# yangbang18/CARE

Measured on AMD Instinct MI355X. Metric: captions/sec (greedy), higher is better.
Workload: dtype bf16; 1 GPU; MSRVTT Transformer/base task=Base feats=ViT modality=ami greedy (BASELINE.json configs[1]): [B,28,128]+[B,28,2048]+[B,28,512] fp32 feats, d=512, V=10547, 29 decoder steps; config_name=msrvtt_base_ami, global_batch=32768, lanes=1, parallelism=batch-sharded dp1 (no data-path collective; all-gather of results), hip_graph=True, absorbed_cross_attention=True, lean_encode=True

## Files before the change

### care_amd/_lib.py

```python
import ctypes
import os
from ctypes import c_char_p, c_float, c_int, c_int64, c_uint64, c_void_p

import torch

CARE_F32, CARE_BF16 = 0, 1
ACT_NONE, ACT_RELU, ACT_GELU = 0, 1, 2
ACT_CODES = {"linear": ACT_NONE, "relu": ACT_RELU, "gelu": ACT_GELU}
ABI_VERSION = 24

_ERRORS = {-1: "CARE_EINVAL (null pointer / bad size)", -2: "CARE_EALIGN (alignment)",
           -3: "CARE_ESHAPE (unsupported shape)", -4: "CARE_EDTYPE (unknown dtype/activation)"}

LIB_PATH = os.environ.get("CARE_HIP_LIB") or os.path.join(os.path.dirname(os.path.abspath(__file__)), "libcare_hip.so")
VARIANT_H16 = {"": "bf16", "f16": "fp16"}

_P, _I, _L, _F, _U = c_void_p, c_int, c_int64, c_float, c_uint64
SIGNATURES = {
    "care_gemm": [_P, _L, _P, _I, _P, _P, _L, _I, _P, _L, _I, _I, _I, _I, _I, _I, _P],
    "care_split3_weight": [_P, _P, _I, _I, _P],
    "care_gemm_split3": [_P, _L, _P, _P, _P, _L, _I, _I, _I, _P],
    "care_gemm_argmax": [_P, _L, _P, _I, _P, _P, _P, _I, _I, _I, _P],
    "care_gemm_bf16": [_P, _L, _I, _P, _P, _P, _L, _I, _P, _L, _I, _I, _I, _I, _I, _I, _P],
    "care_gemm_argmax_bf16": [_P, _L, _I, _P, _P, _P, _P, _P, _P, _I, _I, _I, _P],
    "care_gemm_tile": [_P, _L, _P, _P, _P, _L, _I, _P, _L, _I, _I, _I, _I, _I, _I, _P],
    "care_split2_act": [_P, _L, _P, _I, _I, _P],
    "care_gemm_tile_split3": [_P, _P, _P, _P, _L, _I, _P, _L, _I, _I, _I, _I, _I, _I, _P],
    "care_gemm_tile_split3_argmax": [_P, _P, _P, _P, _P, _I, _I, _I, _P],
    "care_absmax": [_P, _L, _I, _I, _P, _P],
    "care_split_pieces": [_P, _L, _I, _I, _I, _I, _I, _P, _I, _P, _P],
    "care_gemm_tile_split3_scaled": [_P, _P, _P, _P, _L, _I, _I, _I, _P, _P, _I, _P],
    "care_gemm_tile_batched": [_P, _L, _L, _P, _L, _L, _P, _I, _P, _L, _L, _I, _I, _I, _I, _I, _P],
    "care_gemm_tile_argmax": [_P, _L, _P, _P, _P, _P, _P, _P, _I, _I, _I, _P],
    "care_score_partials": [_P, _P, _P, _P, _I, _P, _P, _I, _P],
    "care_label_logits": [_P, _L, _P, _P, _P, _I, _I, _I, _P],
    "care_score_partials_lab": [_P, _P, _P, _I, _P, _P, _P, _I, _P],
    "care_score_logits": [_P, _L, _I, _P, _P, _P, _I, _P],
    "care_greedy_update": [_P, _P, _P, _I, _P, _I, _P, _P, _P, _I, _I, _I, _I, _P],
    "care_greedy_update_embed": [_P, _P, _P, _I, _P, _I, _P, _P, _P, _I, _I, _I, _I, _P, _P, _P, _I, _P, _P, _F,
                                 _P, _P, _L, _I, _P],
    "care_add_ln": [_P, _L, _P, _L, _P, _P, _P, _F, _P, _P, _L, _I, _I, _I, _I, _I, _I, _L, _P],
    "care_gemm_ln": [_P, _L, _I, _P, _P, _P, _L, _P, _P, _P, _F, _P, _P, _L, _I, _I, _I, _I, _I, _I, _P],
    "care_gemm_ln_packed": [_P, _L, _I, _P, _P, _P, _L, _P, _P, _F, _P, _P, _L, _I, _I, _I, _I, _I, _I, _P],
    "care_pack_ln_weight": [_P, _P, _I, _I, _P],
    "care_pack_ln_weight_split": [_P, _P, _I, _I, _P],
    "care_gemm_ln_split": [_P, _L, _P, _P, _P, _P, _F, _P, _P, _L, _I, _I, _I, _I, _I, _I, _P],
    "care_gemm_bf16_splitk": [_P, _L, _I, _P, _P, _P, _L, _L, _I, _I, _I, _P],
    "care_group_mean": [_P, _L, _I, _I, _I, _P, _L, _I, _I, _I, _P],
    "care_concept_finish": [_P, _L, _P, _L, _P, _I, _I, _P],
    "care_concept_topk_embed": [_P, _L, _I, _I, _P, _P, _P, _P, _F, _P, _P, _P, _L, _I, _I, _I, _I, _P],
    "care_embed_ln": [_P, _I, _I, _P, _I, _P, _P, _I, _P, _I, _P, _P, _F, _P, _P, _L, _I, _I, _I, _P],
    "care_attention": [_P, _L, _P, _P, _I, _L, _L, _I, _P, _I, _I, _I, _I, _I, _P, _I, _I, _P, _I, _P, _L,
                       _I, _I, _I, _P],
    "care_attention_seq": [_P, _L, _P, _P, _L, _L, _I, _I, _I, _I, _P, _I, _I, _P, _I, _P, _L, _I, _I, _P],
    "care_attention_latent": [_P, _L, _P, _L, _L, _I, _I, _P, _I, _P, _L, _I, _I, _I, _P],
    "care_head_expand": [_P, _L, _P, _P, _L, _I, _I, _P],
    "care_head_reduce": [_P, _L, _P, _P, _P, _L, _I, _I, _P],
    "care_gemm_argmax_bf16_min": [_P, _L, _I, _P, _P, _P, _P, _I, _I, _I, _I, _P],
    "care_beam_threshold": [_P, _I, _I, _P, _P, _I, _P],
    "care_gemm_argmax_bf16_tiles": [_P, _L, _I, _P, _P, _P, _P, _P, _I, _I, _I, _I, _P],
    "care_beam_sparse_collect": [_P, _L, _P, _P, _P, _P, _P, _P, _I, _P, _P, _I, _I, _I, _P],
    "care_gemm_collect_bf16": [_P, _L, _I, _P, _P, _P, _P, _P, _I, _I, _I, _I, _P],
    "care_beam_pick": [_P, _P, _I, _P, _P, _P, _I, _I, _P, _L, _I, _P, _I, _I, _P, _P, _I, _P],
    "care_gemm_tile_beam": [_P, _L, _P, _P, _P, _P, _I, _I, _I, _P],
    "care_beam_pick_groups": [_P, _P, _P, _I, _I, _P, _L, _P, _I, _I, _P, _P, _I, _P],
    "care_beam_select": [_P, _L, _I, _I, _P, _P, _I, _I, _P],
    "care_ensemble_select": [_P, _I, _L, _I, _I, _P, _P, _I, _P],
    "care_attention_probs": [_P, _L, _P, _I, _L, _L, _I, _I, _I, _I, _P, _I, _I, _P, _I, _P, _I, _I, _P],
    "care_timestamp": [_P, _P],
    "care_decode_resident": [_P, _I, _P, _P, _P, _I, _P, _P, _F, _P, _I, _I, _I, _I, _I, _I, _I, _I, _I, _I, _I, _P, _I, _P, _P, _P,
                             _P, _L, _I, _I, _P],
    "care_decode_resident_beam": [_P, _I, _P, _P, _P, _P, _P, _F, _P, _I, _I, _I, _I, _I, _I, _I, _I, _I, _I, _I, _I, _I, _P, _I,
                                  _P, _P, _P, _P, _P, _P, _P, _P, _I, _P, _L, _I, _I, _P],
    "care_decode_chain_beam": [_P, _I, _P, _P, _P, _P, _P, _F, _P, _I, _I, _I, _I, _I, _I, _I, _I, _I, _I, _I, _I, _I, _I, _P, _I,
                               _P, _P, _P, _P, _P, _P, _P, _P, _I, _P, _L, _I, _P],
    "care_gemm_kn": [_P, _L, _I, _P, _L, _P, _L, _I, _I, _I, _P],
    "care_gemm_kn_splitk": [_P, _L, _I, _P, _L, _P, _L, _L, _I, _I, _I, _I, _P],
    "care_ln_bwd": [_P, _L, _P, _L, _P, _P, _L, _F, _P, _L, _P, _P, _I, _I, _P],
    "care_act": [_P, _P, _P, _L, _I, _P],
    "care_dropout": [_P, _P, _L, _F, _U, _P],
    "care_strided_sum": [_P, _L, _P, _L, _I, _I, _I, _L, _L, _F, _P],
    "care_bcast_rows": [_P, _L, _P, _L, _I, _I, _I, _F, _P],
    "care_add_pos_sem": [_P, _P, _P, _P, _I, _I, _I, _I, _P],
    "care_scatter_add_rows": [_P, _L, _P, _P, _L, _I, _I, _I, _P],
    "care_concept_bwd": [_P, _L, _P, _L, _P, _P, _L, _I, _I, _P],
    "care_attn_pv": [_P, _P, _L, _L, _P, _L, _I, _I, _I, _I, _F, _U, _P],
    "care_attn_bwd": [_P, _L, _P, _P, _L, _L, _P, _P, _L, _P, _L, _P, _P, _L, _L, _P, _I, _I, _I, _I, _I, _F, _U, _P],
    "care_lang_loss_fwd": [_P, _L, _L, _I, _I, _P, _F, _P, _P, _P, _P, _P, _P, _P, _P, _P, _I, _P],
    "care_lang_loss_bwd": [_P, _L, _L, _I, _I, _P, _P, _P, _F, _P, _P, _L, _L, _I, _I, _P],
    "care_noisy_or_bce_fwd": [_P, _L, _P, _L, _P, _P, _P, _P, _I, _I, _P],
    "care_noisy_or_bce_bwd": [_P, _L, _P, _L, _P, _P, _P, _L, _I, _I, _P],
    "care_head_live_rows": [_P, _I, _I, _I, _I, _P, _P, _P, _P, _P],
    "care_gemm_tile_split3_head_stats": [_P, _P, _P, _P, _P, _P, _P, _P, _P, _P, _I, _I, _I, _P],
    "care_head_loss_finish": [_P, _P, _P, _P, _P, _I, _P, _P, _I, _F, _I, _P, _P, _P, _P, _P, _P, _P, _P, _P],
    "care_lang_loss_reduce": [_P, _P, _P, _P, _I, _I, _P, _P, _P, _P],
    "care_head_grad_scale": [_P, _P, _P],
    "care_gemm_tile_split3_head_grad": [_P, _P, _P, _P, _P, _P, _P, _P, _P, _F, _P, _I, _I, _I, _P],
    "care_pieces_transpose": [_P, _I, _I, _I, _I, _I, _P, _P],
    "care_active_slots": [_P, _I, _P, _P, _P],
    "care_gather_rows": [_P, _L, _P, _L, _P, _I, _L, _P],
    "care_scatter_rows": [_P, _L, _P, _L, _P, _I, _L, _P],
    "care_expand_index": [_P, _I, _I, _P, _P],
    "care_remap_rows": [_P, _L, _P, _I, _P],
    "care_beam_advance": [_P, _P, _P, _I, _P, _P, _P, _P, _P, _I, _P, _P, _P, _I, _I, _I, _I, _I, _I, _I, _P],
}
PLAIN = {"care_version": (c_int, []), "care_arch": (c_char_p, []), "care_source_hash": (c_char_p, []),
         "care_build_flags": (c_char_p, []), "care_h16": (c_char_p, []), "care_argmax_parts": (c_int, [c_int]),
         "care_argmax_parts_bf16": (c_int, [c_int, c_int]),
         "care_argmax_parts_tile": (c_int, [c_int]),
         "care_argmax_parts_bf16_min": (c_int, [c_int, c_int, c_int, c_int, c_int]),
# ... 142 lines not shown
```

### care_amd/csrc/heads.hip

```cpp
#include "care_common.h"

#ifndef CARE_HEADS_ST_NT
#define CARE_HEADS_ST_NT 0
#endif
#ifndef CARE_HEADS_LD_AUX
#define CARE_HEADS_LD_AUX 0
#endif

namespace {

__global__ __launch_bounds__(256) void head_expand_kernel(const bf16_t* q, int64_t ldq, const bf16_t* wkt, bf16_t* qt,
                                                          int64_t ldo, int rows) {
  const int lane = threadIdx.x & 63, wave = threadIdx.x >> 6;
  const int fr = lane & 15, fg = lane >> 4;
  const int h = blockIdx.x;
  const bf16_t* wh = wkt + (int64_t)h * 512 * 64 + (int64_t)(wave * 128 + (fr >> 2) * 8 + (fr & 3)) * 64 + fg * 8;
  bf16x8 bw[8][2];
#pragma unroll
  for (int nt = 0; nt < 8; ++nt)
#pragma unroll
    for (int ks = 0; ks < 2; ++ks)
      bw[nt][ks] = *reinterpret_cast<const bf16x8*>(wh + ((nt >> 1) * 32 + (nt & 1) * 4) * 64 + ks * 32);

  const int tiles = (rows + 15) / 16;
  const bf16_t* qh = q + h * 64 + fg * 8;
  auto load_a = [&](int T, bf16x8 (&af)[2]) {
    const bf16_t* src = qh + (int64_t)min(T * 16 + fr, rows - 1) * ldq;
    af[0] = *reinterpret_cast<const bf16x8*>(src);
    af[1] = *reinterpret_cast<const bf16x8*>(src + 32);
  };
  bf16x8 af[2], an[2];
  int T = blockIdx.y;
  if (T < tiles) load_a(T, af);
  for (; T < tiles; T += gridDim.y) {
    const int Tn = T + gridDim.y;
    load_a(min(Tn, tiles - 1), an);
    const int r = T * 16 + fr;
    bf16_t* out = qt + (int64_t)min(r, rows - 1) * ldo + h * 512 + wave * 128 + fg * 8;
#pragma unroll
    for (int k = 0; k < 4; ++k) {
      bf16x8 o;
#pragma unroll
      for (int half = 0; half < 2; ++half) {
        f32x4 acc = f32x4{0.f, 0.f, 0.f, 0.f};
        acc = care_mfma_16x16x32_h16(bw[2 * k + half][0], af[0], acc, 0, 0, 0);
        acc = care_mfma_16x16x32_h16(bw[2 * k + half][1], af[1], acc, 0, 0, 0);
#pragma unroll
        for (int j = 0; j < 4; ++j) o[half * 4 + j] = (bf16_t)acc[j];
      }
      if (CARE_HEADS_ST_NT) __builtin_nontemporal_store(o, reinterpret_cast<bf16x8*>(out + k * 32));
      else *reinterpret_cast<bf16x8*>(out + k * 32) = o;
    }
    af[0] = an[0]; af[1] = an[1];
  }
}

// ... 10 lines not shown
  const bf16_t* wh = wv + (int64_t)(h * 64 + wave * 16 + fr) * 512 + fg * 8;
  bf16x8 bw[16];
#pragma unroll
  for (int ks = 0; ks < 16; ++ks) bw[ks] = *reinterpret_cast<const bf16x8*>(wh + ks * 32);
  f32x4 bias = f32x4{0.f, 0.f, 0.f, 0.f};
  if (bv) bias = *reinterpret_cast<const f32x4*>(bv + h * 64 + wave * 16 + fg * 4);

  const int tiles = (rows + 15) / 16;
  const int nmine = blockIdx.y < tiles ? (tiles - blockIdx.y + gridDim.y - 1) / gridDim.y : 0;
  auto stage = [&](int n, int slot) {
    const int T = blockIdx.y + n * gridDim.y;
#pragma unroll
    for (int j = 0; j < 4; ++j) {
      const int i = wave * 4 + j;
      const unsigned char* g = reinterpret_cast<const unsigned char*>(ct + (int64_t)min(T * 16 + i, rows - 1) * ldc +
                                                                      h * 512) + ((lane ^ i) << 4);
      __builtin_amdgcn_global_load_lds((const __attribute__((address_space(1))) void*)g,
                                       (__attribute__((address_space(3))) void*)(smem + slot * RED_TILE + i * 1024),
                                       16, 0, CARE_HEADS_LD_AUX);
    }
  };
  int roff[4];
#pragma unroll
  for (int r = 0; r < 4; ++r) roff[r] = fr * 1024 + ((((r * 4 + fg) ^ fr) & 15) << 4);

  if (nmine > 0) stage(0, 0);
  if (nmine > 1) stage(1, 1);
  for (int n = 0; n < nmine; ++n) {
    if (n + 1 < nmine) {
      if (n == 0) asm volatile("s_waitcnt vmcnt(4) lgkmcnt(0)" ::: "memory");
      else asm volatile("s_waitcnt vmcnt(5) lgkmcnt(0)" ::: "memory");
    } else {
      asm volatile("s_waitcnt vmcnt(0) lgkmcnt(0)" ::: "memory");
    }
    __builtin_amdgcn_s_barrier();
    __builtin_amdgcn_sched_barrier(0);
    const unsigned char* sb = smem + (n % RED_SLOTS) * RED_TILE;
    f32x4 acc = bias;
#pragma unroll
    for (int ks = 0; ks < 16; ++ks) {
      const bf16x8 a = *reinterpret_cast<const bf16x8*>(sb + roff[ks & 3] + (ks >> 2) * 256);
      acc = care_mfma_16x16x32_h16(bw[ks], a, acc, 0, 0, 0);
    }
    const int T = blockIdx.y + n * gridDim.y;
    bf16x4 o;
#pragma unroll
    for (int j = 0; j < 4; ++j) o[j] = (bf16_t)acc[j];
    *reinterpret_cast<bf16x4*>(ctx + (int64_t)min(T * 16 + fr, rows - 1) * ldo + h * 64 + wave * 16 + fg * 4) = o;
    __builtin_amdgcn_sched_barrier(0);
    if (n + 2 < nmine) stage(n + 2, (n + 2) % RED_SLOTS);
  }
}

}

extern "C" int care_head_expand(const void* q, int64_t ldq, const void* wkt, void* qt, int64_t ldo, int rows, int heads,
                                void* stream) {
  if (!q || !wkt || !qt || rows <= 0 || heads <= 0) return CARE_EINVAL;
  if ((ldq % 8) || (ldo % 8) || !care_aligned16(q) || !care_aligned16(wkt) || !care_aligned16(qt)) return CARE_EALIGN;
  const int tiles = (rows + 15) / 16;
  const int nb = min(tiles, max(1, 1024 / heads));
  hipLaunchKernelGGL(head_expand_kernel, dim3(heads, nb), dim3(256), 0, (hipStream_t)stream,
                     reinterpret_cast<const bf16_t*>(q), ldq, reinterpret_cast<const bf16_t*>(wkt),
                     reinterpret_cast<bf16_t*>(qt), ldo, rows);
  return care_launch_status();
}

extern "C" int care_head_reduce(const void* ct, int64_t ldc, const void* wv, const float* bv, void* ctx, int64_t ldo,
                                int rows, int heads, void* stream) {
  if (!ct || !wv || !ctx || rows <= 0 || heads <= 0) return CARE_EINVAL;
  if ((ldc % 8) || (ldo % 4) || !care_aligned16(ct) || !care_aligned16(wv) || !care_aligned16(ctx) ||
      (bv && !care_aligned16(bv)))
    return CARE_EALIGN;
  const int tiles = (rows + 15) / 16;
  const int nb = min(tiles, max(1, 768 / heads));
  hipLaunchKernelGGL(head_reduce_kernel, dim3(heads, nb), dim3(256), RED_SLOTS * RED_TILE, (hipStream_t)stream,
                     reinterpret_cast<const bf16_t*>(ct), ldc, reinterpret_cast<const bf16_t*>(wv), bv,
                     reinterpret_cast<bf16_t*>(ctx), ldo, rows);
  return care_launch_status();
}
```

### care_amd/engine.py

```python
import collections
import contextlib
import ctypes
import functools
import os
import threading
import weakref
from typing import Dict, List, Optional

import torch

from . import _lib, forms
from ._lib import ACT_CODES, CARE_BF16, CARE_F32, ptr
from .constants import BOS, EOS, PAD
from .engine_beam import BeamMixin
from .engine_decode import DecodeMixin
from .engine_encode import EncodeMixin
from .engine_resident import ResidentMixin
from .engine_util import _LaneOutputs, device_props


_CAPTURE_LOCK = threading.Lock()


class HipEngine(EncodeMixin, DecodeMixin, ResidentMixin, BeamMixin):
# ... 257 lines not shown
        sizes = [int(torch.empty(0, dtype=dt).element_size()) for _, dt in parts]
        offs, total = [], 0
        for (shape, dt), es in zip(parts, sizes):
            offs.append(total)
            n = es
            for s in shape:
                n *= int(s)
            total += (n + 255) // 256 * 256
        blk = self._ws_get(name, (max(total, 256),), torch.uint8)
        out = []
        for (shape, dt), es, off in zip(parts, sizes, offs):
            n = es
            for s in shape:
                n *= int(s)
            out.append(blk[off: off + n].view(dt).view(tuple(shape)))
        return out

    GRAPH_CAPS = {"greedy": 8, "beam": 8, "gseg0": 8, "bseg0": 8, "gseg": 96, "bseg": 96, "tf": 8, "gres": 8}

    def _graph_get(self, key):
        entry = self._graphs.get(key)
        if entry is not None:
            self._graphs.move_to_end(key)
        return entry

    def _graph_put(self, key, entry):
        self._graphs[key] = entry
        self._graphs.move_to_end(key)
        cap = self.GRAPH_CAPS.get(key[0], 8)
        same = [k for k in self._graphs if k[0] == key[0]]
        for k in same[: max(0, len(same) - cap)]:
            del self._graphs[k]

    def _begin_pass(self, plan: forms.PassPlan) -> forms.PassPlan:
        self._gen += 1
        self.plan = plan
        budget = self.ws_budget_bytes
        if budget is None:
            budget = self.ws_budget_bytes = int(0.6 * device_props(self.device).total_memory)
        if self._ws_bytes <= budget:
            return plan
        for key in sorted(self._ws, key=lambda k: self._ws_used.get(k, 0)):
            if self._ws_bytes <= budget // 2 or self._ws_used.get(key, 0) >= self._gen - 1:
                break
            t = self._ws.pop(key)
            self._ws_used.pop(key, None)
            self._ws_bytes -= t.numel() * t.element_size()
        self._graphs.clear()
        self._epoch += 1
        return plan

    MID_TILE_ROWS, VOCAB_TILE_MAX_ROWS = forms.MID_TILE_ROWS, forms.VOCAB_TILE_MAX_ROWS
    BEAM_FUSED_MIN_ROWS, LATENT_MIN_ROWS = forms.BEAM_FUSED_MIN_ROWS, forms.LATENT_MIN_ROWS

    plan_for = forms.plan
    resident_ok, resident_beam_ok, chain_beam_ok = forms.resident_greedy, forms.resident_beam, forms.chain_beam
    small_forms, ln_fusable, tf_fast_ok, lanes_for = forms.small_forms, forms.fuse_ln, forms.tf_fast, forms.lanes
    beam_fused_for, beam_groups_for = forms.beam_fused, forms.beam_groups

    def latent_for(self, rows: int) -> bool:
        return forms.latent(self, rows) and not (self.plan is not None and self.plan.small_beam)

    def _vocab_as(self, rows: int) -> bool:
        return self.plan.vocab_as if self.plan is not None else forms.vocab_as(self, rows)

    @functools.cached_property
    def bf(self) -> bool:
        return self.dtype in ("bf16", "fp16")

    @functools.cached_property
    def as_ok(self) -> bool:
        return self.bf and self.d <= 512 and self.d % 128 == 0

    @functools.cached_property
    def bf_act(self) -> bool:
        return self.bf and self.d % 64 == 0 and self.ff % 64 == 0

    @functools.cached_property
    def latent_capable(self) -> bool:
        if self.H * 64 != self.d or self.H > 16:
            return False
        return (self.as_ok and self.d == 512) or (self.bf_act and self.d in (768, 1024))

    @property
    def latent_ok(self) -> bool:
        return bool(self.latent) and self.latent_capable

    @property
    def act_dtype(self):
        return self.h16 if self.bf_act else torch.float32

    def wsb(self, name: str, shape) -> Optional[torch.Tensor]:
        return self.ws(name + "#bf", shape, self.h16) if self.bf_act else None

    def gemm(self, A, W, bias, out, act=0, out2=None, n_split=None, tag=None, tile=False):
        M, K = A.shape
        N = W.shape[0]
        assert W.shape[1] == K and A.stride(1) == 1 and out.stride(-1) == 1
        tail = (ptr(bias), ptr(out), out.stride(0), self._code(out), ptr(out2),
                out2.stride(0) if out2 is not None else 0, self._code(out2), N if n_split is None else n_split, M, N, K, act)
        if W.dtype == self.h16 and A.dtype == self.h16:
            if K % 64 or A.stride(0) % 8:
                raise ValueError("bf16 A operand needs K % 64 == 0 and a 16-byte aligned row stride (got K = {})".format(K))
            if K <= 512 and K % 128 == 0 and not tile and not forms.mid_tile(M):
                self.call("care_gemm_bf16", ptr(A), A.stride(0), self._code(A), ptr(W), *tail, tag=tag)
            else:
# ... 111 lines not shown
```

### care_amd/engine_decode.py

```python
import ctypes
import functools
import os
from typing import Dict, List, Optional

import torch

from . import _lib, forms
from ._lib import ACT_CODES, CARE_BF16, CARE_F32, ptr
from .constants import BOS, EOS, PAD
from .engine_util import _LaneOutputs


class DecodeMixin:
    def _ctx(self, tag, rows):
        return self.ws(tag + "ctx", (rows, self.d), self.act_dtype)

    def _mha_self_full(self, name, x, xb, seq, pad_tok, causal, tag, aux=None):
        rows, d = x.shape
        w = self.w
        hin, hinb = self._ln_in(x, xb, w[name + "_g"], w[name + "_be"], tag + "sa")
        qkv = self.gemm(hinb if hinb is not None else hin, w[name + "_qkv_w"], w[name + "_qkv_b"],
                        self.ws(tag + "qkv", (rows, 3 * d)))
        ctx = self.attention(qkv, qkv[:, d:], qkv[:, 2 * d:], self._ctx(tag, rows), seq * 3 * d, 3 * d,
                             seq, seq, causal=causal, seq=seq, pad_tok=pad_tok)
# ... 219 lines not shown
            self.call("care_score_logits", ptr(lg), lg.stride(0), self.V, ptr(lab32), ptr(logp), ptr(pred), rows)
        return logp.view(N, t), pred.view(N, t)

    def metrics_step(self, feats: List[torch.Tensor], input_ids: torch.Tensor, labels: torch.Tensor):
        feats = self._prep_feats(feats)
        plan = self._begin_pass(self.plan_for(feats[0].shape[0], rows=input_ids.numel(), lean=not self.has_concepts))
        if (not self.has_concepts and self.tf_fast_ok(input_ids.shape[1], False) and
                os.environ.get("CARE_TF_OVERLAP", "1") != "0"):
            if getattr(self, "_tf_side", None) is None:
                self._tf_side = torch.cuda.Stream(device=self.device)
            side, cur = self._tf_side, torch.cuda.current_stream()
            side.wait_stream(cur)
            with torch.cuda.stream(side):
                enc = self.encode(feats, lean=True)
                ckv = self.cross_kv(enc["encoder_hidden_states"], tag="tf_ckv", tile=True)
            self._tf_ckv_ready = (ckv, side)
            try:
                logp, pred = self.score_teacher_forced(input_ids, labels, enc["encoder_hidden_states"], None, plan=plan)
            finally:
                self._tf_ckv_ready = None
                cur.wait_stream(side)
            return logp, pred, enc
        enc = self.encode(feats, lean=not self.has_concepts)
        logp, pred = self.score_teacher_forced(input_ids, labels, enc["encoder_hidden_states"], enc.get("semantic_hidden_states"),
                                               sem_embs=enc.get("semantic_embs"), plan=plan)
        return logp, pred, enc

    def _decode_step(self, t, N, rows_per_clip, tok, anc, sem, ckv, skv, Lk, tag, akv=None, embedded=False):
        w, d, T = self.w, self.d, self.T
        x, xb = self.ws(tag + "x0", (N, d)), self.wsb(tag + "x0", (N, d))
        if not embedded:
            self.call("care_embed_ln", ptr(tok), tok.stride(0), t - 1, ptr(anc), anc.stride(0) if anc is not None else 0,
                 ptr(w["word"]), ptr(w["pos"]), t - 1, ptr(sem), rows_per_clip, ptr(w["emb_g"]), ptr(w["emb_be"]),
                 self.eps, ptr(x), ptr(xb), d, N, 1, d)
        g = lambda f32, b16: b16 if b16 is not None else f32
        fuse_ln = self.plan.fuse_ln
        for li in range(self.n_layers):
            nm = "d{}_sa".format(li)
            cache = skv[li]
            q = self.ws(tag + "q", (N, d))
            hin, hinb = self._ln_in(x, xb, w[nm + "_g"], w[nm + "_be"], tag + "sa")
            self.gemm(g(hin, hinb), w[nm + "_qkv_w"], w[nm + "_qkv_b"], q, out2=cache[:, t - 1, :], n_split=d,
                      tag="step_qkv_gemm")
            flat = cache.view(N * T, 2 * d)
            ctx = self.attention(q, flat, flat[:, d:], self._ctx(tag, N), T * 2 * d, 2 * d, 1, t, anc=anc,
                                 pad_tok=tok, tag="step_self_attn")
            x1, x1b = self.ws(tag + "x1", (N, d)), self.wsb(tag + "x1", (N, d))
            self._dense_ln(ctx, nm, x, x1, x1b, tag, "step_dxd", "step_add_ln")
            nm = "d{}_ca".format(li)
            hb = w["d{}_hb".format(li)]
            x1in, x1inb = self._ln_in(x1, x1b, w[nm + "_g"], w[nm + "_be"], tag + "ca")
            if isinstance(ckv, tuple):
                H = self.H
                q2 = self.gemm(x1inb, w[nm + "_q_w"], w[nm + "_q_b"], self.ws(tag + "q2b", (N, d), self.h16),
                               tag="step_dxd_gemm", tile=self.plan.q_tile)
                qt = self.ws(tag + "qt", (N, H * d), self.h16)
                if d == 512:
                    self.call("care_head_expand", ptr(q2), d, ptr(w[nm + "_wkt"]), ptr(qt), H * d, N, H, tag="step_head_expand")
                else:
                    self.call("care_gemm_tile_batched", ptr(q2), d, 64, ptr(w[nm + "_wkt"]), 64, d * 64, None, 0, ptr(qt), H * d, d,
                         CARE_BF16, H, N, d, 64, tag="step_head_expand")
                ct = self.ws(tag + "ct", (N, H * d), self.h16)
                self.call("care_attention_latent", ptr(qt), H * d, ptr(ckv[li]), Lk * d, d, rows_per_clip, Lk, ptr(hb),
                     hb.stride(0) if hb is not None else 0, ptr(ct), H * d, N, H, d, tag="step_cross_attn")
                ctx = self._ctx(tag, N)
                if d == 512:
                    self.call("care_head_reduce", ptr(ct), H * d, ptr(w[nm + "_v_w"]), ptr(w[nm + "_v_b"]), ptr(ctx), d, N, H,
                         tag="step_head_reduce")
                else:
                    self.call("care_gemm_tile_batched", ptr(ct), H * d, d, ptr(w[nm + "_v_w"]), d, 64 * d, ptr(w[nm + "_v_b"]), 64,
                         ptr(ctx), d, 64, CARE_BF16, H, N, 64, d, tag="step_head_reduce")
            else:
                q2 = self.gemm(g(x1in, x1inb), w[nm + "_q_w"], w[nm + "_q_b"], self.ws(tag + "q2", (N, d)),
                               tag="step_dxd_gemm")
                kv = ckv[li]
                ctx = self.attention(q2, kv, kv[:, d:], self._ctx(tag, N), Lk * 2 * d, 2 * d, rows_per_clip, Lk,
                                     bias=hb, tag="step_cross_attn")
            x2, x2b = self.ws(tag + "x2", (N, d)), self.wsb(tag + "x2", (N, d))
            self._dense_ln(ctx, nm, x1, x2, x2b, tag, "step_dxd", "step_add_ln")
            if self.attr_att:
                x2, x2b = self._attr_block(li, x2, x2b, akv, rows_per_clip, tag)
            x, xb = self.ws(tag + "x3_%d" % (li & 1), (N, d)), self.wsb(tag + "x3_%d" % (li & 1), (N, d))
            bf16_only = (li == self.n_layers - 1 and xb is not None and fuse_ln and self.as_ok and
                         self.ff % 512 == 0 and self.ff >= 1024)
            self._ffn("d{}_ffn".format(li), x2, x2b, None if bf16_only else x, xb, tag, gemm_tag="step_ffn_gemm",
                      fuse=fuse_ln)
            if bf16_only:
                x = None
        if self.pre_ln:
            xf, xfb = self.ws(tag + "xfin", (N, d)), self.wsb(tag + "xfin", (N, d))
            self.add_ln(x, None, w["dec_g"], w["dec_be"], xf, xfb, tag="step_add_ln")
            x, xb = xf, xfb
        return x, xb

    def _greedy_steps(self, v, t0, t1, last):
        n, T, d, w = v["n"], self.T, self.d, self.w
        parts = self.vocab_parts(n)
        pmax, psum = self.ws(v["tag"] + "pmax", (n, parts)), self.ws(v["tag"] + "psum", (n, parts))
        pidx = self.ws(v["tag"] + "pidx", (n, parts), torch.int32)
        for t in range(t0, t1 + 1):
            x, xb = self._decode_step(t, n, 1, v["fed"], None, v["sem"], v["ckv"], v["skv"], v["Lk"], v["tag"], akv=v["akv"],
                                      embedded=t > 1)
            self.vocab_argmax(x, xb, n, pmax, pidx, psum)
            update = (ptr(pmax), ptr(pidx), ptr(psum), parts, ptr(v["fed"]), T + 1, ptr(v["score"]), ptr(v["length"]),
                      ptr(v["fin"]), t, T, EOS, n)
            if t < last:
                self.call("care_greedy_update_embed", *update, ptr(w["word"]), ptr(w["pos"]), ptr(v["sem"]), 1, ptr(w["emb_g"]),
                          ptr(w["emb_be"]), self.eps, ptr(v["x0"]), ptr(v["x0b"]), d, d, tag="step_update_embed")
            else:
                self.call("care_greedy_update", *update)

    def _greedy_init(self, v):
        v["fed"].zero_(); v["fed"][:, 0] = BOS
        v["score"].zero_(); v["length"].zero_(); v["fin"].zero_()
# ... 202 lines not shown
```

### care_amd/forms.py

```python
import dataclasses
from typing import Optional

MID_TILE_ROWS = (1280, 16384)
FUSED_SMALL_MIN_ROWS = 5376
VOCAB_TILE_MAX_ROWS = 2048
LN_FUSED_MIN_ROWS = 10240
FFN2_TILE_MIN_ROWS = 1 << 30
Q_TILE_MIN_ROWS = 8192
LATENT_MIN_ROWS = 1
BEAM_FUSED_MIN_ROWS = 8192
BEAM_GROUPS_MIN_ROWS = 1
RESIDENT_MAX_V = 64 * 64 * 4
RESIDENT_WIDE_MAX_ROWS = 128
RESIDENT_BEAM_MAX = 8
RESIDENT_WIDE_BEAM_MAX_ROWS = 256


def resident_model_ok(m) -> bool:
    if m.pre_ln or not (m.bf and m.wt == m.h16 and m.T <= 128 and m.n_layers <= 4 and (not m.attr_att or m.topk <= 128) and
                        m.V <= RESIDENT_MAX_V and m.Lk <= 128):
        return False
    if m.d == 512:
        return bool(m.as_ok and m.ff in (512, 1024, 2048))
    return bool(m.d in (768, 1024) and m.ff == 4 * m.d and m.bf_act)


def resident_fits(m, kind: str, rows: int, per_tile: int = 1) -> bool:
    if rows >= m._resident_refused.get(kind, 1 << 30):
        return False
    return m._cus is None or ((rows + 15) // 16 + per_tile - 1) // per_tile <= m._cus // 8 * 8


def resident_greedy(m, clips: int) -> bool:
    return bool(0 < clips <= m.resident_max_rows and resident_model_ok(m) and (m.d == 512 or clips <= RESIDENT_WIDE_MAX_ROWS) and
                resident_fits(m, "greedy", clips))


def _beam_model_ok(m, bm: int, need: int, max_bm: int) -> bool:
    return bool(1 < bm <= max_bm and need >= 1 and resident_model_ok(m) and m.T <= 63 and m.V >= 16 * RESIDENT_BEAM_MAX)


def resident_beam(m, clips: int, bm: int, need: int) -> bool:
    rows = clips * bm
    if not (0 < rows <= m.resident_beam_max_rows and _beam_model_ok(m, bm, need, RESIDENT_BEAM_MAX)):
        return False
    if m.d != 512 and rows > (RESIDENT_WIDE_BEAM_MAX_ROWS if m.d <= 768 else min(160, RESIDENT_WIDE_BEAM_MAX_ROWS)):
        return False
    return resident_fits(m, "beam", rows, 2 if rows > 512 else 1)


def chain_beam(m, clips: int, bm: int, need: int) -> bool:
    return bool(0 < clips * bm <= m.chain_beam_max_rows and m.d == 512 and _beam_model_ok(m, bm, need, 5))


def small_forms(m, clips: int) -> bool:
    return bool(0 < clips <= m.resident_max_rows and m.as_ok and m.d == 512)


def latent(m, rows: int) -> bool:
    return bool(m.latent_ok and rows >= m.LATENT_MIN_ROWS)


def fuse_ln(m, rows: int) -> bool:
    return bool(m.as_ok and m.d == 512 and not m.pre_ln and rows >= LN_FUSED_MIN_ROWS)


def vocab_as(m, rows: int) -> bool:
    return bool(m.as_ok and rows > VOCAB_TILE_MAX_ROWS)


def mid_tile(rows: int) -> bool:
    return MID_TILE_ROWS[0] <= rows < MID_TILE_ROWS[1]


def beam_fused(m, rows: int) -> bool:
    return bool(m.as_ok and rows >= m.BEAM_FUSED_MIN_ROWS)


def beam_groups(m, rows: int, bm: int) -> bool:
    return bool(m.bf_act and not beam_fused(m, rows) and bm <= 8 and rows >= BEAM_GROUPS_MIN_ROWS and
                128 <= m.V <= 16384 and m.d % 64 == 0)


def tf_fast(m, t: int, want_aux: bool) -> bool:
    return bool(m.as_ok and m.d == 512 and not want_aux and t <= 32 and not m.pre_ln)


def lanes(m, clips: int) -> int:
    return max(1, min(int(m.lanes), clips))


@dataclasses.dataclass(frozen=True)
class PassPlan:
    decode: str
    clips: int
    bm: Optional[int]
    need: int
    rows: int
    small: bool
    small_beam: bool
    latent: bool
    fuse_ln: bool
    vocab_as: bool
    q_tile: bool
    mid_tile: bool
    beam_select: str
    sparse_second_pass: bool
    lean: bool
    early_exit: bool
    lanes: int


def plan(m, clips: int, bm: Optional[int] = None, need: int = 1, lean: bool = False, early_exit: Optional[bool] = None,
         rows: Optional[int] = None, n_lanes: int = 1) -> PassPlan:
    beam = bm is not None
    ee = bool(m.early_exit if early_exit is None else early_exit)
    decode = "multi"
    if rows is None and n_lanes == 1:
        if resident_beam(m, clips, bm, need) if beam else resident_greedy(m, clips):
            decode = "resident"
        elif beam and chain_beam(m, clips, bm, need):
            decode = "chain"
    rows = clips * (bm or 1) if rows is None else rows
    small, multi = small_forms(m, clips), decode != "resident"
    fused = beam and multi and beam_fused(m, rows)
    return PassPlan(
        decode=decode, clips=clips, bm=bm, need=need, rows=rows,
        small=(beam and not multi) or (small and (beam or not multi)), small_beam=beam and small,
        latent=latent(m, rows) and not (beam and small), fuse_ln=fuse_ln(m, rows), vocab_as=vocab_as(m, rows),
        q_tile=m.d == 512 and rows >= Q_TILE_MIN_ROWS, mid_tile=mid_tile(rows),
        beam_select=("fused" if fused else "groups" if beam_groups(m, rows, bm) else "logits") if beam and multi else "",
        sparse_second_pass=fused and m.d == 512, lean=bool(lean and m.lean_ok), early_exit=ee and n_lanes == 1, lanes=n_lanes)


def graph_key(name: str, plan: PassPlan, feats=(), *site) -> tuple:
    return (name, plan) + site + (tuple(f.data_ptr() for f in feats), tuple(tuple(f.shape) for f in feats))
```

### include/care_hip.h

```cpp
#ifndef CARE_HIP_H
#define CARE_HIP_H

#include <stdint.h>

#ifdef __cplusplus
extern "C" {
#endif

#define CARE_ABI_VERSION 24

enum { CARE_F32 = 0, CARE_BF16 = 1 };
enum { CARE_ACT_NONE = 0, CARE_ACT_RELU = 1, CARE_ACT_GELU = 2 };
enum {
  CARE_EINVAL = -1,
  CARE_EALIGN = -2,
  CARE_ESHAPE = -3,
  CARE_EDTYPE = -4
};

int care_version(void);

const char* care_arch(void);

const char* care_source_hash(void);
const char* care_build_flags(void);
const char* care_h16(void);

int care_gemm(const float* A, int64_t lda, const void* W, int wdtype, const float* bias,
              void* C0, int64_t ldc0, int c0_dtype, void* C1, int64_t ldc1, int c1_dtype,
              int n_split, int M, int N, int K, int act, void* stream);

int care_argmax_parts(int N);
int care_gemm_argmax(const float* A, int64_t lda, const void* W, int wdtype,
                     float* pmax, int32_t* pidx, float* psum, int M, int N, int K, void* stream);

int care_split3_weight(const float* W, void* W3, int N, int K, void* stream);
int care_gemm_split3(const float* A, int64_t lda, const void* W3, const float* bias, float* C,
                     int64_t ldc, int M, int N, int K, void* stream);

int care_gemm_bf16(const void* A, int64_t lda, int a_dtype, const void* W, const float* bias,
                   void* C0, int64_t ldc0, int c0_dtype, void* C1, int64_t ldc1, int c1_dtype,
                   int n_split, int M, int N, int K, int act, void* stream);
int care_argmax_parts_bf16(int M, int N);
int care_gemm_bf16_splitk(const void* A, int64_t lda, int a_dtype, const void* W,
                          const float* bias, float* C, int64_t ldc, int64_t slab_stride,
                          int M, int N, int K, void* stream);
int care_gemm_argmax_bf16(const void* A, int64_t lda, int a_dtype, const void* W, float* pmax,
                          int32_t* pidx, float* psum, const int32_t* labels, float* plab,
                          int M, int N, int K, void* stream);

int care_split2_act(const float* A, int64_t lda, void* A2, int M, int K, void* stream);
int care_gemm_tile_split3(const void* A2, const void* W3, const float* bias, void* C0, int64_t ldc0, int c0_dtype,
                          void* C1, int64_t ldc1, int c1_dtype, int n_split, int M, int N, int K, int act,
                          void* stream);
int care_absmax(const float* A, int64_t lda, int M, int K, void* slot, void* stream);
int care_split_pieces(const float* src, int64_t ld, int rows, int K, int transposed, int slabs, int ks, void* out,
                      int pieces, const void* amax, void* stream);
int care_gemm_tile_split3_scaled(const void* A2, const void* W3, const float* bias, float* C, int64_t ldc, int M, int N,
                                 int K, const void* amax_a, const void* amax_b, int slabs, void* stream);
int care_gemm_tile_split3_argmax(const void* A2, const void* W3, float* pmax, int32_t* pidx, float* psum, int M,
                                 int N, int K, void* stream);
int care_gemm_tile(const void* A, int64_t lda, const void* W, const float* bias, void* C0, int64_t ldc0,
// ... 40 lines not shown

int care_pack_ln_weight(const void* W, void* W_packed, int N, int K, void* stream);
int care_gemm_ln_packed(const void* A, int64_t lda, int a_dtype, const void* W_packed,
                        const float* bias, const float* res, int64_t ldres, const float* gamma,
                        const float* beta, float eps, float* out, void* out_bf16, int64_t ldo,
                        int M, int N, int K, int grp, int out_grp_rows, int out_row_off,
                        void* stream);

int care_pack_ln_weight_split(const float* W, void* W_split, int N, int K, void* stream);
int care_gemm_ln_split(const void* A, int64_t lda, const void* W_split, const float* bias,
                       const float* gamma, const float* beta, float eps, float* out,
                       void* out_bf16, int64_t ldo, int M, int N, int K, int grp,
                       int out_grp_rows, int out_row_off, void* stream);

int care_group_mean(const float* x, int64_t ldx, int in_grp_rows, int in_row_off, int grp,
                    float* out, int64_t ldo, int col_off, int groups, int d, void* stream);

int care_concept_finish(const float* scores, int64_t lds, float* preds, int64_t ldp,
                        float* avg, int B, int k, void* stream);

int care_concept_topk_embed(const float* preds, int64_t ldp, int k, int topk,
                            const float* word, const float* pos, const float* gamma,
                            const float* beta, float eps, int64_t* labels, float* out,
                            void* out_bf16, int64_t ldo, int out_grp_rows, int out_row_off,
                            int B, int d, void* stream);

int care_embed_ln(const int32_t* tokens, int tok_stride, int tok_off, const int32_t* anc,
                  int anc_stride, const float* word, const float* pos, int pos0,
                  const float* sem, int sem_div, const float* gamma, const float* beta,
                  float eps, float* out, void* out_bf16, int64_t ldo, int rows, int seq, int d,
                  void* stream);

int care_attention(const float* Q, int64_t ldq, const void* K, const void* V, int kv_dtype,
                   int64_t kv_batch_stride, int64_t kv_row_stride, int rows_per_kv,
                   const int32_t* anc, int anc_stride, int nkeys, int causal, int seq,
                   int causal_off, const int32_t* pad_tok, int pad_stride, int pad_id,
                   const float* bias, int bias_ld, void* ctx, int64_t ldctx, int ctx_dtype,
                   int rows, int heads, void* stream);

int care_attention_seq(const void* Q, int64_t ldq, const void* K, const void* V, int64_t kv_batch_stride,
                       int64_t kv_row_stride, int seqs_per_kv, int nkeys, int causal, int seq,
                       const int32_t* pad_tok, int pad_stride, int pad_id, const float* bias, int bias_ld,
                       void* ctx, int64_t ldctx, int nseq, int heads, void* stream);

int care_attention_latent(const void* qt, int64_t ldq, const void* mem, int64_t mem_batch_stride,
                          int64_t mem_row_stride, int rows_per_kv, int nkeys, const float* bias,
                          int bias_ld, void* ct, int64_t ldc, int rows, int heads, int d,
                          void* stream);

int care_head_expand(const void* q, int64_t ldq, const void* wkt, void* qt, int64_t ldo, int rows,
                     int heads, void* stream);
int care_head_reduce(const void* ct, int64_t ldc, const void* wv, const float* bv, void* ctx,
                     int64_t ldo, int rows, int heads, void* stream);

int care_beam_select(const float* logits, int64_t ldl, int V, int bm, float* cand_val,
                     int32_t* cand_idx, int rows, int waves_per_row, void* stream);

int care_ensemble_select(const float* const* logits, int n_models, int64_t ldl, int V, int bm, float* cand_val,
                         int32_t* cand_idx, int rows, void* stream);

int care_argmax_parts_bf16_min(int M, int N, int K, int a_dtype, int min_parts);
int care_gemm_argmax_bf16_min(const void* A, int64_t lda, int a_dtype, const void* W, float* pmax,
                              int32_t* pidx, float* psum, int M, int N, int K, int min_parts,
                              void* stream);
int care_beam_threshold(const float* pmax, int parts, int bm, float* thr, int32_t* cnt, int rows,
                        void* stream);
int care_gemm_collect_bf16(const void* A, int64_t lda, int a_dtype, const void* W, const float* thr,
                           int32_t* cnt, float* cval, int32_t* cidx, int cap, int M, int N, int K,
                           void* stream);
int care_beam_sparse_applies(int M, int N, int K, int a_dtype);
int care_gemm_argmax_bf16_tiles(const void* A, int64_t lda, int a_dtype, const void* W, float* pmax,
                                int32_t* pidx, float* psum, float* tile_max, int M, int N, int K,
                                int min_parts, void* stream);
int care_beam_sparse_collect(const void* A, int64_t lda, const void* W, const float* tile_max,
                             const float* thr, int32_t* cnt, float* cval, int32_t* cidx, int cap,
                             int32_t* tcount, int32_t* tlist, int M, int N, int K, void* stream);
int care_beam_pick(const float* pmax, const float* psum, int parts, const int32_t* cnt,
                   const float* cval, const int32_t* cidx, int cap, int bm, const void* A, int64_t lda,
                   int a_dtype, const void* W, int V, int K, float* cand_val, int32_t* cand_idx,
                   int rows, void* stream);

int care_gemm_tile_beam(const void* A, int64_t lda, const void* W, float* pmax, float* psum, float* gmax, int M,
                        int N, int K, void* stream);
int care_beam_pick_groups(const float* pmax, const float* psum, const float* gmax, int parts, int bm, const void* A,
                          int64_t lda, const void* W, int V, int K, float* cand_val, int32_t* cand_idx, int rows,
                          void* stream);

int care_beam_advance(const float* cand_val, const int32_t* cand_idx, float* scores, int bm,
                      int32_t* tokphys, const int32_t* anc_old, int32_t* anc_new,
                      int32_t* done, int32_t* n_fin, int fin_cap, float* fin_score,
                      int32_t* fin_len, int32_t* fin_hyp, int t, int max_steps, int need,
                      int eos_id, int V, int stride, int B, void* stream);

int care_attention_probs(const float* Q, int64_t ldq, const void* K, int kv_dtype,
                         int64_t kv_batch_stride, int64_t kv_row_stride, int rows_per_kv, int nkeys,
                         int causal, int seq, const int32_t* pad_tok, int pad_stride, int pad_id,
                         const float* bias, int bias_ld, float* probs, int rows, int heads,
                         void* stream);

int care_active_slots(const int32_t* finished, int n, int32_t* idx, int32_t* count, void* stream);
int care_gather_rows(const void* src, int64_t src_stride_bytes, void* dst, int64_t dst_stride_bytes,
                     const int32_t* idx, int n, int64_t row_bytes, void* stream);
int care_scatter_rows(const void* src, int64_t src_stride_bytes, void* dst, int64_t dst_stride_bytes,
                      const int32_t* idx, int n, int64_t row_bytes, void* stream);
int care_expand_index(const int32_t* idx_c, int m, int bm, int32_t* idx_r, void* stream);
int care_remap_rows(int32_t* anc, int64_t n, const int32_t* cmap, int bm, void* stream);
// ... 102 lines not shown
```

Measured before the change: 670,000 captions/s.

## Fuse cross-attention Q projection into per-head latent expansion kernel

New measurement: 660,400 captions/s. -1.4%, worse.

```diff
diff --git a/care_amd/_lib.py b/care_amd/_lib.py
--- a/care_amd/_lib.py
+++ b/care_amd/_lib.py
@@ -7,7 +7,7 @@
 CARE_F32, CARE_BF16 = 0, 1
 ACT_NONE, ACT_RELU, ACT_GELU = 0, 1, 2
 ACT_CODES = {"linear": ACT_NONE, "relu": ACT_RELU, "gelu": ACT_GELU}
-ABI_VERSION = 24
+ABI_VERSION = 25
 
 _ERRORS = {-1: "CARE_EINVAL (null pointer / bad size)", -2: "CARE_EALIGN (alignment)",
            -3: "CARE_ESHAPE (unsupported shape)", -4: "CARE_EDTYPE (unknown dtype/activation)"}
@@ -56,6 +56,7 @@
     "care_attention_latent": [_P, _L, _P, _L, _L, _I, _I, _P, _I, _P, _L, _I, _I, _I, _P],
     "care_head_expand": [_P, _L, _P, _P, _L, _I, _I, _P],
     "care_head_reduce": [_P, _L, _P, _P, _P, _L, _I, _I, _P],
+    "care_q_head_expand": [_P, _L, _P, _P, _P, _P, _L, _I, _I, _P],
     "care_gemm_argmax_bf16_min": [_P, _L, _I, _P, _P, _P, _P, _I, _I, _I, _I, _P],
     "care_beam_threshold": [_P, _I, _I, _P, _P, _I, _P],
     "care_gemm_argmax_bf16_tiles": [_P, _L, _I, _P, _P, _P, _P, _P, _I, _I, _I, _I, _P],
diff --git a/care_amd/csrc/heads.hip b/care_amd/csrc/heads.hip
--- a/care_amd/csrc/heads.hip
+++ b/care_amd/csrc/heads.hip
@@ -2,6 +2,9 @@
 
 #ifndef CARE_HEADS_ST_NT
 #define CARE_HEADS_ST_NT 0
+#endif
+#ifndef CARE_QX_ST_NT
+#define CARE_QX_ST_NT 1
 #endif
 #ifndef CARE_HEADS_LD_AUX
 #define CARE_HEADS_LD_AUX 0
@@ -118,6 +121,103 @@
   }
 }
 
+constexpr int QX_ROWB = 144;
+constexpr int QX_LDS = RED_SLOTS * RED_TILE + 16 * QX_ROWB;
+
+__global__ __launch_bounds__(256, 3) void q_head_expand_kernel(const bf16_t* x, int64_t ldx, const bf16_t* wq, const float* bq,
+                                                            const bf16_t* wkt, bf16_t* qt, int64_t ldo, int rows, int heads) {
+  extern __shared__ __attribute__((aligned(16))) unsigned char smem[];
+  unsigned char* const xch = smem + RED_SLOTS * RED_TILE;
+  const int lane = threadIdx.x & 63;
+  const int wave = __builtin_amdgcn_readfirstlane(threadIdx.x >> 6);
+  const int fr = lane & 15, fg = lane >> 4;
+  const int slot8 = blockIdx.x >> 3;
+  const int h = slot8 % heads, y = (slot8 / heads) * 8 + (blockIdx.x & 7), stride = gridDim.x / heads;
+  const bf16_t* wh = wkt + (int64_t)h * 512 * 64 + (int64_t)(wave * 128 + (fr >> 2) * 8 + (fr & 3)) * 64 + fg * 8;
+  bf16x8 bw[8][2];
+#pragma unroll
+  for (int nt = 0; nt < 8; ++nt)
+#pragma unroll
+    for (int ks = 0; ks < 2; ++ks)
+      bw[nt][ks] = *reinterpret_cast<const bf16x8*>(wh + ((nt >> 1) * 32 + (nt & 1) * 4) * 64 + ks * 32);
+  const bf16_t* wqh = wq + (int64_t)(h * 64 + wave * 16 + fr) * 512 + fg * 8;
+  bf16x8 bq_w[16];
+#pragma unroll
+  for (int ks = 0; ks < 16; ++ks) bq_w[ks] = *reinterpret_cast<const bf16x8*>(wqh + ks * 32);
+  f32x4 bias = f32x4{0.f, 0.f, 0.f, 0.f};
+  if (bq) bias = *reinterpret_cast<const f32x4*>(bq + h * 64 + wave * 16 + fg * 4);
+
+  const int tiles = (rows + 15) / 16;
+  const int nmine = y < tiles ? (tiles - y + stride - 1) / stride : 0;
+  auto stage = [&](int n, int slot) {
+    const int T = y + n * stride;
+#pragma unroll
+    for (int j = 0; j < 4; ++j) {
+      const int i = wave * 4 + j;
+      const unsigned char* g = reinterpret_cast<const unsigned char*>(x + (int64_t)min(T * 16 + i, rows - 1) * ldx) + ((lane ^ i) << 4);
+      __builtin_amdgcn_global_load_lds((const __attribute__((address_space(1))) void*)g,
+                                       (__attribute__((address_space(3))) void*)(smem + slot * RED_TILE + i * 1024),
+                                       16, 0, 0);
+    }
+  };
+  int roff[4];
+#pragma unroll
+  for (int r = 0; r < 4; ++r) roff[r] = fr * 1024 + ((((r * 4 + fg) ^ fr) & 15) << 4);
+  unsigned char* const xw = xch + fr * QX_ROWB + (wave * 16 + fg * 4) * 2;
+  const unsigned char* const xr = xch + fr * QX_ROWB + fg * 16;
+
+  if (nmine > 0) stage(0, 0);
+  if (nmine > 1) stage(1, 1);
+#pragma nounroll
+  for (int n = 0; n < nmine; ++n) {
+    if (n + 1 < nmine) {
+      if (n >= 2) asm volatile("s_waitcnt vmcnt(12) lgkmcnt(0)" ::: "memory");
+      else asm volatile("s_waitcnt vmcnt(4) lgkmcnt(0)" ::: "memory");
+    } else {
+      if (n >= 2) asm volatile("s_waitcnt vmcnt(8) lgkmcnt(0)" ::: "memory");
+      else asm volatile("s_waitcnt vmcnt(0) lgkmcnt(0)" ::: "memory");
+    }
+    __builtin_amdgcn_s_barrier();
+    __builtin_amdgcn_sched_barrier(0);
+    if (n + 2 < nmine) stage(n + 2, (n + 2) % RED_SLOTS);
+    __builtin_amdgcn_sched_barrier(0);
+    const unsigned char* sb = smem + (n % RED_SLOTS) * RED_TILE;
+    f32x4 qa = f32x4{0.f, 0.f, 0.f, 0.f};
+#pragma unroll
+    for (int ks = 0; ks < 16; ++ks) {
+      const bf16x8 a = *reinterpret_cast<const bf16x8*>(sb + roff[ks & 3] + (ks >> 2) * 256);
+      qa = care_mfma_16x16x32_h16(bq_w[ks], a, qa, 0, 0, 0);
+    }
+    bf16x4 qo;
+#pragma unroll
+    for (int j = 0; j < 4; ++j) qo[j] = (bf16_t)(qa[j] + bias[j]);
+    *reinterpret_cast<bf16x4*>(xw) = qo;
+    asm volatile("s_waitcnt lgkmcnt(0)" ::: "memory");
+    __builtin_amdgcn_s_barrier();
+    __builtin_amdgcn_sched_barrier(0);
+    bf16x8 af[2];
+    af[0] = *reinterpret_cast<const bf16x8*>(xr);
+    af[1] = *reinterpret_cast<const bf16x8*>(xr + 64);
+    const int T = y + n * stride;
+    bf16_t* out = qt + (int64_t)min(T * 16 + fr, rows - 1) * ldo + h * 512 + wave * 128 + fg * 8;
+#pragma unroll
+    for (int k = 0; k < 4; ++k) {
+      bf16x8 o;
+#pragma unroll
+      for (int half = 0; half < 2; ++half) {
+        f32x4 acc = f32x4{0.f, 0.f, 0.f, 0.f};
+        acc = care_mfma_16x16x32_h16(bw[2 * k + half][0], af[0], acc, 0, 0, 0);
+        acc = care_mfma_16x16x32_h16(bw[2 * k + half][1], af[1], acc, 0, 0, 0);
+#pragma unroll
+        for (int j = 0; j < 4; ++j) o[half * 4 + j] = (bf16_t)acc[j];
+      }
+      if (CARE_QX_ST_NT) __builtin_nontemporal_store(o, reinterpret_cast<bf16x8*>(out + k * 32));
+      else *reinterpret_cast<bf16x8*>(out + k * 32) = o;
+    }
+    __builtin_amdgcn_sched_barrier(0);
+  }
+}
+
 }
 
 extern "C" int care_head_expand(const void* q, int64_t ldq, const void* wkt, void* qt, int64_t ldo, int rows, int heads,
@@ -145,3 +245,18 @@
                      reinterpret_cast<bf16_t*>(ctx), ldo, rows);
   return care_launch_status();
 }
+
+extern "C" int care_q_head_expand(const void* x, int64_t ldx, const void* wq, const float* bq, const void* wkt, void* qt,
+                                  int64_t ldo, int rows, int heads, void* stream) {
+  if (!x || !wq || !wkt || !qt || rows <= 0 || heads <= 0) return CARE_EINVAL;
+  if ((ldx % 8) || (ldo % 8) || !care_aligned16(x) || !care_aligned16(wq) || !care_aligned16(wkt) || !care_aligned16(qt) ||
+      (bq && !care_aligned16(bq)))
+    return CARE_EALIGN;
+  if (ldx < 512 || ldo < (int64_t)heads * 512) return CARE_ESHAPE;
+  const int tiles = (rows + 15) / 16;
+  const int nb = (min(tiles, max(1, 768 / heads)) + 7) & ~7;
+  hipLaunchKernelGGL(q_head_expand_kernel, dim3(nb * heads), dim3(256), QX_LDS, (hipStream_t)stream,
+                     reinterpret_cast<const bf16_t*>(x), ldx, reinterpret_cast<const bf16_t*>(wq), bq,
+                     reinterpret_cast<const bf16_t*>(wkt), reinterpret_cast<bf16_t*>(qt), ldo, rows, heads);
+  return care_launch_status();
+}
diff --git a/care_amd/engine.py b/care_amd/engine.py
--- a/care_amd/engine.py
+++ b/care_amd/engine.py
@@ -333,6 +333,7 @@
 
     MID_TILE_ROWS, VOCAB_TILE_MAX_ROWS = forms.MID_TILE_ROWS, forms.VOCAB_TILE_MAX_ROWS
     BEAM_FUSED_MIN_ROWS, LATENT_MIN_ROWS = forms.BEAM_FUSED_MIN_ROWS, forms.LATENT_MIN_ROWS
+    XATTN_FUSED_MIN_ROWS = forms.XATTN_FUSED_MIN_ROWS
 
     plan_for = forms.plan
     resident_ok, resident_beam_ok, chain_beam_ok = forms.resident_greedy, forms.resident_beam, forms.chain_beam
diff --git a/care_amd/engine_decode.py b/care_amd/engine_decode.py
--- a/care_amd/engine_decode.py
+++ b/care_amd/engine_decode.py
@@ -295,14 +295,19 @@
             x1in, x1inb = self._ln_in(x1, x1b, w[nm + "_g"], w[nm + "_be"], tag + "ca")
             if isinstance(ckv, tuple):
                 H = self.H
-                q2 = self.gemm(x1inb, w[nm + "_q_w"], w[nm + "_q_b"], self.ws(tag + "q2b", (N, d), self.h16),
-                               tag="step_dxd_gemm", tile=self.plan.q_tile)
-                qt = self.ws(tag + "qt", (N, H * d), self.h16)
-                if d == 512:
-                    self.call("care_head_expand", ptr(q2), d, ptr(w[nm + "_wkt"]), ptr(qt), H * d, N, H, tag="step_head_expand")
+                if self.plan.xattn_fused:
+                    qt = self.ws(tag + "qt", (N, H * d), self.h16)
+                    self.call("care_q_head_expand", ptr(x1inb), x1inb.stride(0), ptr(w[nm + "_q_w"]), ptr(w[nm + "_q_b"]),
+                         ptr(w[nm + "_wkt"]), ptr(qt), H * d, N, H, tag="step_head_expand")
                 else:
-                    self.call("care_gemm_tile_batched", ptr(q2), d, 64, ptr(w[nm + "_wkt"]), 64, d * 64, None, 0, ptr(qt), H * d, d,
-                         CARE_BF16, H, N, d, 64, tag="step_head_expand")
+                    q2 = self.gemm(x1inb, w[nm + "_q_w"], w[nm + "_q_b"], self.ws(tag + "q2b", (N, d), self.h16),
+                                   tag="step_dxd_gemm", tile=self.plan.q_tile)
+                    qt = self.ws(tag + "qt", (N, H * d), self.h16)
+                    if d == 512:
+                        self.call("care_head_expand", ptr(q2), d, ptr(w[nm + "_wkt"]), ptr(qt), H * d, N, H, tag="step_head_expand")
+                    else:
+                        self.call("care_gemm_tile_batched", ptr(q2), d, 64, ptr(w[nm + "_wkt"]), 64, d * 64, None, 0, ptr(qt), H * d,
+                             d, CARE_BF16, H, N, d, 64, tag="step_head_expand")
                 ct = self.ws(tag + "ct", (N, H * d), self.h16)
                 self.call("care_attention_latent", ptr(qt), H * d, ptr(ckv[li]), Lk * d, d, rows_per_clip, Lk, ptr(hb),
                      hb.stride(0) if hb is not None else 0, ptr(ct), H * d, N, H, d, tag="step_cross_attn")
diff --git a/care_amd/forms.py b/care_amd/forms.py
--- a/care_amd/forms.py
+++ b/care_amd/forms.py
@@ -1,5 +1,5 @@
 import dataclasses
-from typing import Optional
+from typing import ClassVar, Optional
 
 MID_TILE_ROWS = (1280, 16384)
 FUSED_SMALL_MIN_ROWS = 5376
@@ -7,6 +7,7 @@
 LN_FUSED_MIN_ROWS = 10240
 FFN2_TILE_MIN_ROWS = 1 << 30
 Q_TILE_MIN_ROWS = 8192
+XATTN_FUSED_MIN_ROWS = 16384
 LATENT_MIN_ROWS = 1
 BEAM_FUSED_MIN_ROWS = 8192
 BEAM_GROUPS_MIN_ROWS = 1
@@ -73,6 +74,10 @@
     return MID_TILE_ROWS[0] <= rows < MID_TILE_ROWS[1]
 
 
+def xattn_fused(m, rows: int) -> bool:
+    return bool(m.as_ok and m.d == 512 and latent(m, rows) and rows >= m.XATTN_FUSED_MIN_ROWS)
+
+
 def beam_fused(m, rows: int) -> bool:
     return bool(m.as_ok and rows >= m.BEAM_FUSED_MIN_ROWS)
 
@@ -109,6 +114,11 @@
     lean: bool
     early_exit: bool
     lanes: int
+    xattn_fused: ClassVar[bool] = False
+
+
+class XattnFusedPlan(PassPlan):
+    xattn_fused: ClassVar[bool] = True
 
 
 def plan(m, clips: int, bm: Optional[int] = None, need: int = 1, lean: bool = False, early_exit: Optional[bool] = None,
@@ -124,7 +134,8 @@
     rows = clips * (bm or 1) if rows is None else rows
     small, multi = small_forms(m, clips), decode != "resident"
     fused = beam and multi and beam_fused(m, rows)
-    return PassPlan(
+    cls = XattnFusedPlan if multi and not (beam and small) and xattn_fused(m, rows) else PassPlan
+    return cls(
         decode=decode, clips=clips, bm=bm, need=need, rows=rows,
         small=(beam and not multi) or (small and (beam or not multi)), small_beam=beam and small,
         latent=latent(m, rows) and not (beam and small), fuse_ln=fuse_ln(m, rows), vocab_as=vocab_as(m, rows),
diff --git a/include/care_hip.h b/include/care_hip.h
--- a/include/care_hip.h
+++ b/include/care_hip.h
@@ -7,7 +7,7 @@
 extern "C" {
 #endif
 
-#define CARE_ABI_VERSION 24
+#define CARE_ABI_VERSION 25
 
 enum { CARE_F32 = 0, CARE_BF16 = 1 };
 enum { CARE_ACT_NONE = 0, CARE_ACT_RELU = 1, CARE_ACT_GELU = 2 };
@@ -154,6 +154,9 @@
                      int heads, void* stream);
 int care_head_reduce(const void* ct, int64_t ldc, const void* wv, const float* bv, void* ctx,
                      int64_t ldo, int rows, int heads, void* stream);
+
+int care_q_head_expand(const void* x, int64_t ldx, const void* wq, const float* bq, const void* wkt,
+                       void* qt, int64_t ldo, int rows, int heads, void* stream);
 
 int care_beam_select(const float* logits, int64_t ldl, int V, int bm, float* cand_val,
                      int32_t* cand_idx, int rows, int waves_per_row, void* stream);
```
